# samtools/htslib

Hardware: NVIDIA H100
Metric: BGZF inflate + CRAM rANS decode GB/s at 1/2/4/8 H100 vs reference CPU (higher is better)
Workload: dtype u8

## Files before the change

htslib_b200/csrc/rans_nx16.cu:

```cuda
#include "hgpu_internal.h"
#include <stdio.h>

namespace {

constexpr uint32_t RANS_L = 1u << 15;
constexpr int SM_F      = 0;
constexpr int SM_CUM    = 1024;
constexpr int SM_ROWOF  = 2064;
constexpr int SM_SYMOF  = 2320;
constexpr int SM_RING   = 2576;
constexpr int SM_TAB    = 3088;
constexpr uint32_t GTAB_BYTES = 256u * 4096u + 256u * 256u * 4u;
constexpr uint32_t TBLBUF_BYTES = 256u * 1024u;

struct WarpScratch {
    uint8_t *tmp;
    uint8_t *planes;
    uint8_t *meta;
    uint8_t *tblbuf;
    uint8_t *gtab;
    uint32_t max_out;
    uint8_t *tab_base;
    uint32_t tab_cap;
    int pass;
    mutable bool defer;
    struct Hook *hook;
    bool compact = false;
};

struct Hook {
    int mode;
    bool taken;
    uint32_t order, N, shift, lb, ncol, ipos, U, R, row0, tab_bytes;
    const uint8_t *in; uint32_t in_len;
    uint8_t *out;
    uint8_t *lut; uint32_t *fb;
    uint16_t *Fcap;
};
constexpr int HOOK_X32 = 1, HOOK_N4 = 2;
constexpr int RC_HOOKED = 2;


__device__ int vget(const uint8_t *p, const uint8_t *end, uint32_t &v)
{
    const uint8_t *s = p;
    uint32_t acc = 0;
    uint8_t c;
    if (end - p >= 6) {
        int budget = 5;
        do { c = *p++; acc = (acc << 7) | (c & 0x7f); } while ((c & 0x80) && budget-- > 0);
    } else {
        if (p >= end) { v = 0; return 0; }
        do { c = *p++; acc = (acc << 7) | (c & 0x7f); } while ((c & 0x80) && p < end);
    }
    v = acc;
    return (int)(p - s);
}

__device__ int read_alphabet(const uint8_t *p, const uint8_t *end, uint32_t *F)
{
    const uint8_t *s = p;
    int run = 0, sym;
    if (p >= end) return 0;
    sym = *p++;
    if (sym == 0 && p + 2 >= end) return (int)(p - s);
    for (;;) {
        F[sym] = 1;
        if (p >= end) return 0;
        if (run == 0 && sym + 1 == *p) {
            if (p + 1 >= end) return 0;
            sym = *p++;
            run = *p++;
        } else if (run) {
// ... 355 lines not shown
            __syncwarp();
            ncol++;
        }
    }
    if (p == in) return -1;
    if (tot != 0 && tot != 4096) {
        int sh = 0;
        while (tot < 4096) { tot *= 2; sh++; }
        __syncwarp();
        for (uint32_t k = lane; k < ncol; k += 32) F[k] <<= sh;
        __syncwarp();
    }
    bool bad = false;
    for (uint32_t k = lane; k < ncol; k += 32) bad |= F[k] > 4096u;
    if (__any_sync(0xffffffffu, bad)) return -1;
    if (warp_cumsum(F, cum, (int)ncol) != 4096u) return -1;
    if (ncol == 0) return -1;
    Table t = place_table(smem, ws, 1, ncol, 12);
    if (ws.defer) return -1;
    fill_row(t, 0, F, cum, symof, N == 32);
    __syncwarp();
    uint32_t R;
    if (load_states(p, end, N, R)) return -1;
    uint32_t ipos = (uint32_t)(p - in) + 4 * N;
    if (top && ws.hook && t.in_smem && ws.hook->mode == (N == 32 ? HOOK_X32 : HOOK_N4)) {
        Hook &h = *ws.hook;
        if (h.Fcap && ncol <= 16) {
            __syncwarp();
            if (lane < 16) h.Fcap[lane] = lane < ncol ? (uint16_t)F[lane] : (uint16_t)0;
            if (lane == 0) h.Fcap[256] = 0;
            __syncwarp();
        }
        h.taken = true; h.order = 0; h.N = N; h.shift = 12; h.ncol = ncol; h.ipos = ipos; h.U = U; h.R = R; h.row0 = 0;
        h.in = in; h.in_len = in_len; h.out = out; h.lut = t.lut; h.fb = t.fb; h.lb = t.lb;
        h.tab_bytes = table_bytes(1, ncol, t.lb);
        return RC_HOOKED;
    }
    if (t.lb != t.shift) loop_order0<true, true>(smem, t, in, in_len, ipos, out, U, N, R);
    else if (t.in_smem)  loop_order0<true>(smem, t, in, in_len, ipos, out, U, N, R);
    else                 loop_order0<false>(smem, t, in, in_len, ipos, out, U, N, R);
    __syncwarp();
    return 0;
}

__device__ int dec_order1(uint8_t *smem, const WarpScratch &ws, const uint8_t *in, uint32_t in_len,
                          uint8_t *out, uint32_t U, uint32_t N, bool top = false)
{
    uint32_t *F = reinterpret_cast<uint32_t *>(smem + SM_F);
    uint32_t *cum = reinterpret_cast<uint32_t *>(smem + SM_CUM);
    uint8_t *rowof = smem + SM_ROWOF;
    uint8_t *symof = smem + SM_SYMOF;
    const uint32_t lane = hgpu_lane();
    if (in_len < (N == 4 ? 16u : 4u * N)) return -1;
    const uint8_t *p = in, *end = in + in_len, *tend = end, *after_tab = nullptr;
    const uint32_t shift = *p >> 4;
    if (*p++ & 1) {
        uint32_t usz, csz;
        p += vget(p, end, usz);
        p += vget(p, end, csz);
        if (csz > (uint32_t)(end - p)) return -1;
        if (usz > TBLBUF_BYTES) return -1;
        after_tab = p + csz;
        if (dec_order0(smem, ws, p, csz, ws.tblbuf, usz, 4)) return -1;
        __syncwarp();
        __threadfence_block();
        p = ws.tblbuf;
        tend = ws.tblbuf + usz;
    }
    if (shift != 10 && shift != 12) return -1;
    __syncwarp();
    for (int j = lane; j < 256; j += 32) { F[j] = 0; rowof[j] = 0xff; }
    __syncwarp();
    int n = read_alphabet(p, tend, F);
    if (!n) return -1;
    p += n;
    if (p >= tend) return -1;
    __syncwarp();
    uint32_t ncol = 0;
    bool zero_in_a0 = F[0] != 0;
    for (int j = 0; j < 256; j++) {
        if (F[j] || j == 0) {
            __syncwarp();
            if (lane == 0) { rowof[j] = (uint8_t)ncol; symof[ncol] = (uint8_t)j; }
            ncol++;
        }
    }
    __syncwarp();
    Table t = place_table(smem, ws, ncol, ncol, shift);
    if (ws.defer) return -1;
    const uint32_t total = 1u << shift;
    const uint8_t *rows_at = p;
build_rows:
    uint16_t *Fcap = (top && ws.hook && N == 32 && ncol <= 16) ? ws.hook->Fcap : nullptr;
    if (Fcap) {
        __syncwarp();
        for (uint32_t k = lane; k < 17 * 16; k += 32) Fcap[k] = k >= 256 ? (uint16_t)1 : (uint16_t)0;
        __syncwarp();
    }
    for (uint32_t r = 0; r < ncol; r++) {
        if (t.lb != shift && (r == 0 && !zero_in_a0)) goto need_full;
        if (r == 0 && !zero_in_a0) { fill_null_row(t, 0); continue; }
        const uint8_t *q = p;
        uint32_t T = 0;
        int dz = 0;
        if (q == tend) return -1;
        __syncwarp();
        for (uint32_t k = lane; k < ncol; k += 32) F[k] = 0;
        __syncwarp();
        for (uint32_t k = zero_in_a0 ? 0 : 1; k < ncol && q < tend; k++) {
            uint32_t f;
            if (dz) { f = 0; dz--; }
            else {
                q += vget(q, tend, f);
                if (f == 0) { if (q >= tend) return -1; dz = *q++; }
            }
            if (lane == 0) F[k] = f;
            T += f;
        }
        __syncwarp();
        if (q == p) return -1;
        p = q;
        if (!T && t.lb != shift) goto need_full;
        if (!T) { fill_null_row(t, r); continue; }
        if (T != total) {
            int sh = 0; uint32_t tt = T;
            while (tt < total) { tt *= 2; sh++; }
            for (uint32_t k = lane; k < ncol; k += 32) F[k] <<= sh;
            __syncwarp();
        }
        bool bad = false;
        for (uint32_t k = lane; k < ncol; k += 32) bad |= F[k] > total;
        if (__any_sync(0xffffffffu, bad)) return -1;
        if (warp_cumsum(F, cum, (int)ncol) != total) return -1;
        fill_row(t, r, F, cum, symof, false);
        if (Fcap) {
            if (lane < ncol) Fcap[r * 16 + lane] = (uint16_t)F[lane];
            if (lane == 0) Fcap[256 + r] = 0;
        }
        __syncwarp();
    }
    if (false) {
need_full:
        __syncwarp();
        t = place_table(smem, ws, ncol, ncol, shift, true);
        if (ws.defer) return -1;
        p = rows_at;
        goto build_rows;
    }
    __syncwarp();
    if (!t.in_smem) __threadfence_block();
    if (after_tab) p = after_tab;
    uint32_t R;
    if (load_states(p, end, N, R)) return -1;
    uint32_t ipos = (uint32_t)(p - in) + 4 * N;
    if (top && ws.hook && t.in_smem && ws.hook->mode == (N == 32 ? HOOK_X32 : HOOK_N4)) {
        Hook &h = *ws.hook;
        h.taken = true; h.order = 1; h.N = N; h.shift = shift; h.ncol = ncol; h.ipos = ipos; h.U = U; h.R = R; h.row0 = 0;
        h.in = in; h.in_len = in_len; h.out = out; h.lut = t.lut; h.fb = t.fb; h.lb = t.lb;
        h.tab_bytes = table_bytes(ncol, ncol, t.lb);
        return RC_HOOKED;
    }
    if (t.lb != shift) {
        if (N == 32) loop_order1<true, true, true>(smem, t, in, in_len, ipos, out, U, N, R, 0);
        else         loop_order1<true, false, true>(smem, t, in, in_len, ipos, out, U, N, R, 0);
    } else if (t.in_smem) {
        if (N == 32) loop_order1<true, true>(smem, t, in, in_len, ipos, out, U, N, R, 0);
        else         loop_order1<true, false>(smem, t, in, in_len, ipos, out, U, N, R, 0);
    } else           loop_order1<false, false>(smem, t, in, in_len, ipos, out, U, N, R, 0);
    __syncwarp();
    return 0;
}

__device__ int unpack_meta(const uint8_t *d, uint32_t len, uint8_t *map, int &per_byte)
{
    if (!len) return 0;
    uint32_t n = d[0] ? d[0] : 256, j = 1, c = 0;
    if (n <= 1) per_byte = 0;
    else if (n <= 2) per_byte = 8;
    else if (n <= 4) per_byte = 4;
    else if (n <= 16) per_byte = 2;
    else { per_byte = 1; return 1; }
    if (len <= 1) return 0;
    do { map[c++] = d[j++]; } while (c < n && j < len);
    return c < n ? 0 : (int)j;
}

__device__ int unpack(const uint8_t *d, uint64_t len, uint8_t *out, uint64_t olen, int per_byte,
                      const uint8_t *map)
{
    const uint32_t lane = hgpu_lane();
    if (per_byte == 1) { for (uint64_t i = lane; i < len; i += 32) out[i] = d[i]; return 0; }
    if (per_byte == 0) { for (uint64_t i = lane; i < olen; i += 32) out[i] = map[0]; return 0; }
// ... 408 lines not shown
        job = __shfl_sync(0xffffffffu, job, 0);
        if (job >= n) break;
        uint32_t got = 0;
        int rc = dec_4x8(gtab, in + in_off[job], in_len[job], out + out_off[job], out_len[job], got);
        __syncwarp();
        if (hgpu_lane() == 0) { status[job] = rc ? HGPU_RANS_ERR : HGPU_OK; got_len[job] = rc ? 0 : got; }
    }
}

}

static uint32_t g_f32_smem[64];

static uint32_t f32_smem(hgpu_ctx *ctx) { int d = ctx->device; return d >= 0 && d < 64 && g_f32_smem[d] ? g_f32_smem[d] : F32_SMEM + F32_LUT; }

static int rans_attrs(hgpu_ctx *ctx)
{
    static bool done[64];
    int dev = ctx->device;
    if (dev >= 0 && dev < 64 && done[dev]) return 0;
    {
        uint32_t *d_o = nullptr, base = 0;
        if (hgpu_check(cudaMalloc(&d_o, 4), "probe alloc")) return -1;
        rans_smem_probe_kernel<<<1, 32, 1024>>>(d_o);
        cudaError_t e = cudaMemcpy(&base, d_o, 4, cudaMemcpyDeviceToHost);
        cudaFree(d_o);
        if (hgpu_check(e, "smem probe")) return -1;
        uint32_t lut0 = (base + F32_WARPS * F32_RING + F32_LUT - 1) & ~(F32_LUT - 1);
        if (dev >= 0 && dev < 64) g_f32_smem[dev] = lut0 + F32_WARPS * (F32_LUT + F32_FB) - base;
    }
    if (hgpu_check(cudaFuncSetAttribute(rans_nx16_decode_kernel<1>, cudaFuncAttributeMaxDynamicSharedMemorySize, (int)(SM_TAB + 18 * 1024)), "rans smem attr") ||
        hgpu_check(cudaFuncSetAttribute(rans_prep32_kernel, cudaFuncAttributeMaxDynamicSharedMemorySize, (int)PREP_SMEM), "rans smem attr") ||
        hgpu_check(cudaFuncSetAttribute(rans_tile4_kernel, cudaFuncAttributeMaxDynamicSharedMemorySize, (int)T4_SMEM), "rans smem attr") ||
        hgpu_check(cudaFuncSetAttribute(rans_fast32_kernel, cudaFuncAttributeMaxDynamicSharedMemorySize, (int)f32_smem(ctx)), "rans smem attr"))
        return -1;
    if (dev >= 0 && dev < 64) done[dev] = true;
    return 0;
}

extern "C" uint32_t hgpu_rans_nx16_wave_size(hgpu_ctx *ctx)
{
    if (!ctx) return 0;
    if (cudaSetDevice(ctx->device) != cudaSuccess || rans_attrs(ctx)) return 0;
    int per_sm = 0;
    if (cudaOccupancyMaxActiveBlocksPerMultiprocessor(&per_sm, rans_fast32_kernel, F32_WARPS * 32, f32_smem(ctx)) != cudaSuccess) return 0;
    return (uint32_t)ctx->sm_count * (uint32_t)(per_sm < 1 ? 1 : per_sm) * F32_WARPS;
}

int hgpu_launch_rans_nx16(hgpu_ctx *ctx, const uint8_t *d_in, const uint64_t *d_in_off,
                          const uint32_t *d_in_len, uint32_t n, uint8_t *d_out,
                          const uint64_t *d_out_off, const uint32_t *d_out_len,
                          uint32_t *d_got_len, int32_t *d_status, uint32_t max_out_len,
                          cudaStream_t st)
{
    if (n == 0) return HGPU_OK;
    if (hgpu_check(cudaSetDevice(ctx->device), "cudaSetDevice") || rans_attrs(ctx)) return HGPU_ERR_CUDA;
    const uint32_t smem1 = SM_TAB + 18 * 1024;
    int per_prep = 0, per_t4 = 0, per_f32 = 0, per_gen = 0;
    if (hgpu_check(cudaOccupancyMaxActiveBlocksPerMultiprocessor(&per_prep, rans_prep32_kernel, 32, PREP_SMEM), "rans occupancy") ||
        hgpu_check(cudaOccupancyMaxActiveBlocksPerMultiprocessor(&per_t4, rans_tile4_kernel, 32, T4_SMEM), "rans occupancy") ||
        hgpu_check(cudaOccupancyMaxActiveBlocksPerMultiprocessor(&per_f32, rans_fast32_kernel, F32_WARPS * 32, f32_smem(ctx)), "rans occupancy") ||
        hgpu_check(cudaOccupancyMaxActiveBlocksPerMultiprocessor(&per_gen, rans_nx16_decode_kernel<1>, 32, smem1), "rans occupancy"))
        return HGPU_ERR_CUDA;
    auto grid_of = [&](int per_sm, uint32_t units) {
        uint32_t g = (uint32_t)ctx->sm_count * (uint32_t)(per_sm < 1 ? 1 : per_sm);
        return g > units ? (units ? units : 1u) : g;
    };
    const uint32_t g_prep = grid_of(per_prep, n), g_t4 = grid_of(per_t4, (n + 7) / 8 + 1);
    const uint32_t g_f32 = grid_of(per_f32, (n + F32_WARPS - 1) / F32_WARPS), g_gen = grid_of(per_gen, n);
    const size_t lists_b = ((size_t)2 * n * 4 + 255) & ~(size_t)255;
    const size_t jobs_b = (((size_t)n * sizeof(FastJob)) + 255) & ~(size_t)255;
    const size_t fixed = lists_b + 256 + jobs_b;
    const size_t mo = ((size_t)max_out_len + 255) & ~(size_t)255;
    const size_t per_small = TBLBUF_BYTES;
    const size_t per_gen_b = (3 * mo + 1024 + TBLBUF_BYTES + GTAB_BYTES + 255) & ~(size_t)255;
    size_t area = per_small * g_prep;
    if (per_small * g_t4 > area) area = per_small * g_t4;
    if (per_gen_b * g_gen > area) area = per_gen_b * g_gen;
    int rc = hgpu_ensure_scratch(ctx, fixed + area);
    if (rc) return rc;
    uint8_t *sc = ctx->d_scratch;
    uint32_t *list32 = reinterpret_cast<uint32_t *>(sc), *list4 = list32 + n;
    uint32_t *counts = reinterpret_cast<uint32_t *>(sc + lists_b);
    FastJob *jobs = reinterpret_cast<FastJob *>(sc + lists_b + 256);
    uint8_t *percta = sc + fixed;
    uint32_t *c_prep = hgpu_take_counter(ctx, st), *c_t4 = hgpu_take_counter(ctx, st), *c_f32 = hgpu_take_counter(ctx, st);
    uint32_t *c_gen = hgpu_take_counter(ctx, st), *njobs = hgpu_take_counter(ctx, st);
    if (!c_prep || !c_t4 || !c_f32 || !c_gen || !njobs) return HGPU_ERR_CUDA;
    rans_classify_kernel<<<1, 1024, 0, st>>>(d_in, d_in_off, d_in_len, n, d_status, list32, list4, counts);
    rans_prep32_kernel<<<g_prep, 32, PREP_SMEM, st>>>(d_in, d_in_off, d_in_len, list32, counts, d_out, d_out_off, d_out_len,
                                                      d_got_len, d_status, percta, per_small, max_out_len, jobs, njobs, c_prep);
    rans_tile4_kernel<<<g_t4, 32, T4_SMEM, st>>>(d_in, d_in_off, d_in_len, list4, counts, d_out, d_out_off, d_out_len,
                                                 d_got_len, d_status, percta, per_small, max_out_len, c_t4);
    rans_fast32_kernel<<<g_f32, F32_WARPS * 32, f32_smem(ctx), st>>>(jobs, njobs, d_in, d_in_off, d_in_len, d_out, d_out_off, d_out_len,
                                                                     d_status, c_f32, f32_smem(ctx));
    rans_nx16_decode_kernel<1><<<g_gen, 32, smem1, st>>>(d_in, d_in_off, d_in_len, n, d_out, d_out_off, d_out_len,
                                                         d_got_len, d_status, percta, per_gen_b,
                                                         max_out_len, 18 * 1024, c_gen);
    hgpu_count_launch(5);
    return hgpu_check(cudaGetLastError(), "rans launch");
}

extern "C" int hgpu_rans4x8_decode_batch_dev(hgpu_ctx *ctx, const uint8_t *d_in, const uint64_t *d_in_off,
        const uint32_t *d_in_len, uint32_t n, uint8_t *d_out, const uint64_t *d_out_off, const uint32_t *d_out_len,
        uint32_t *d_got_len, int32_t *d_status, void *stream)
{
    if (!ctx) { hgpu_set_error("null context"); return HGPU_ERR_ARG; }
    if (n == 0) return HGPU_OK;
    cudaStream_t st = stream ? (cudaStream_t)stream : ctx->stream;
    uint32_t grid = (uint32_t)ctx->sm_count * 16u;
    if (grid > n) grid = n;
    size_t per_cta = (GTAB_BYTES + 1024 + 255) & ~(size_t)255;
    int rc = hgpu_ensure_scratch(ctx, per_cta * grid);
    if (rc) return rc;
    uint32_t *counter = hgpu_take_counter(ctx, st);
    if (!counter) return HGPU_ERR_CUDA;
    rans_4x8_decode_kernel<<<grid, 32, 0, st>>>(d_in, d_in_off, d_in_len, n, d_out, d_out_off, d_out_len, d_got_len,
                                                d_status, ctx->d_scratch, per_cta, counter);
    hgpu_count_launch();
    return hgpu_check(cudaGetLastError(), "rans4x8 launch");
}
```

htslib_b200/csrc/rans_nx16_fast.cuh:

```cuda

constexpr int32_t RANS_PENDING = 3;

__global__ void __launch_bounds__(1024)
rans_classify_kernel(const uint8_t *__restrict__ in, const uint64_t *__restrict__ in_off,
                     const uint32_t *__restrict__ in_len, uint32_t n, int32_t *status,
                     uint32_t *list32, uint32_t *list4, uint32_t *counts )
{
    __shared__ uint32_t wsum[2][32];
    __shared__ uint32_t base[2];
    const uint32_t tid = threadIdx.x, lane = tid & 31, warp = tid >> 5;
    if (tid < 2) base[tid] = 0;
    __syncthreads();
    for (uint32_t i0 = 0; i0 < n; i0 += 1024) {
        uint32_t i = i0 + tid;
        int cls = 0;
        if (i < n) {
            uint32_t len = in_len[i];
            if (len >= 2) {
                uint8_t fmt = in[in_off[i]];
                if (!(fmt & 0xe8)) cls = (fmt & 0x04) ? 1 : 2;
            }
            status[i] = cls ? RANS_PENDING : RANS_DEFERRED;
        }
        uint32_t b1 = __ballot_sync(0xffffffffu, cls == 1), b2 = __ballot_sync(0xffffffffu, cls == 2);
        if (lane == 0) { wsum[0][warp] = __popc(b1); wsum[1][warp] = __popc(b2); }
        __syncthreads();
        uint32_t o1 = base[0], o2 = base[1];
        for (uint32_t w = 0; w < warp; w++) { o1 += wsum[0][w]; o2 += wsum[1][w]; }
        if (cls == 1) list32[o1 + __popc(b1 & hgpu_lanemask_lt())] = i;
        if (cls == 2) list4[o2 + __popc(b2 & hgpu_lanemask_lt())] = i;
        __syncthreads();
        if (tid == 0) {
            uint32_t t1 = 0, t2 = 0;
            for (int w = 0; w < 32; w++) { t1 += wsum[0][w]; t2 += wsum[1][w]; }
            base[0] += t1; base[1] += t2;
        }
        __syncthreads();
    }
    if (tid == 0) { counts[0] = base[0]; counts[1] = base[1]; }
}

struct __align__(16) FastJob {
    uint32_t job, ipos, shift, ncol, order, s0, U, hdr;
    uint32_t slen, pad[3];
    uint8_t  symof[8];
    uint8_t  ctx[32];
    uint32_t R[32];
    uint32_t prev[32];
    uint16_t F[64];
};

constexpr uint32_t F32_WARPS = 4, F32_LUT = 4096, F32_FB = 128, F32_RING = 768;
constexpr uint32_t F32_SMEM = F32_WARPS * (F32_LUT + F32_FB + F32_RING);
constexpr uint32_t F32_HEAD = 4;
constexpr uint32_t F32_MIN_U = 32 * 64;

__device__ bool fast32_emit(uint8_t *smem, const Hook &h, uint32_t job, uint32_t hdr, FastJob *jobs, uint32_t *njobs)
{
    const uint32_t lane = hgpu_lane();
    const uint16_t *Fc = h.Fcap;
    if (h.ncol > 16 || h.U < F32_MIN_U || h.lb != h.shift) return false;
    uint32_t emit = 0, nullrows = 0;
    const uint32_t rows = h.order ? h.ncol : 1;
    for (uint32_t r = 0; r < rows; r++) {
        if (h.order && Fc[256 + r]) { nullrows |= 1u << r; continue; }
        for (uint32_t k = 0; k < h.ncol; k++) if (Fc[r * 16 + k]) emit |= 1u << k;
    }
    const uint32_t ne = __popc(emit);
    if (ne == 0 || ne > 8) return false;
    if (h.order) {
        if ((ne << h.shift) > F32_LUT || ne > 4) return false;
        if (nullrows & emit) return false;
    }
    if (h.order && (nullrows & 1u)) return false;
    const uint8_t *symof = smem + SM_SYMOF;
    uint32_t R = h.R, ipos = h.ipos, acc = 0, krow = 0;
    if (h.order) {
        const uint32_t mask = (1u << h.shift) - 1, seg = h.U / 32;
        uint8_t *op = h.out + (size_t)lane * seg;
        uint8_t *ring = smem + SM_RING;
        WordRing wr;
        ring_init(ring, wr, h.in, h.in_len, ipos);
        uint32_t lrow = h.row0 << h.shift, frow = h.row0 * h.ncol;
        for (uint32_t s = 0; s < F32_HEAD; s++) {
            ring_ensure(ring, wr, ipos, 64);
            uint32_t m = R & mask;
            uint32_t k = h.lut[lrow + m];
            uint32_t e = h.fb[frow + k];
            uint32_t q = R >> h.shift;
            R = (e >> 20) * q + q + m - ((e >> 8) & 0xfffu);
            acc = __funnelshift_l(acc, e, 24);
            lrow = k << h.shift; frow = k * h.ncol; krow = k;
            renorm_safe(R, true, ring, wr, ipos, h.in_len);
            op[s] = (uint8_t)(acc >> 24);
        }
        __syncwarp();
        if (__any_sync(0xffffffffu, !(emit >> krow & 1u))) return false;
    }
    uint32_t slot = 0;
    if (lane == 0) slot = atomicAdd(njobs, 1u);
    slot = __shfl_sync(0xffffffffu, slot, 0);
    FastJob *fj = jobs + slot;
    if (lane == 0) {
        fj->job = job; fj->ipos = ipos; fj->shift = h.shift; fj->ncol = ne; fj->order = h.order;
        fj->s0 = h.order ? F32_HEAD : 0; fj->U = h.U; fj->hdr = hdr; fj->slen = h.in_len;
        uint32_t e = 0;
        for (uint32_t k = 0; k < h.ncol; k++) if (emit >> k & 1) fj->symof[e++] = symof[k];
        for (; e < 8; e++) fj->symof[e] = 0;
    }
    fj->R[lane] = R;
    fj->prev[lane] = acc;
    fj->ctx[lane] = (uint8_t)__popc(emit & ((1u << krow) - 1u));
    for (uint32_t idx = lane; idx < 64; idx += 32) {
        uint32_t re = idx >> 3, ke = idx & 7;
        uint16_t v = 0;
        if (re < (h.order ? ne : 1u) && ke < ne) {
            uint32_t r = h.order ? (uint32_t)__fns(emit, 0, re + 1) : 0u, k = (uint32_t)__fns(emit, 0, ke + 1);
            v = Fc[r * 16 + k];
        }
        fj->F[idx] = v;
    }
    return true;
}

__device__ __forceinline__ void lds_v2(uint32_t a, uint32_t &x, uint32_t &y)
{ asm volatile("ld.shared.v2.u32 {%0, %1}, [%2];" : "=r"(x), "=r"(y) : "r"(a) : "memory"); }
__device__ __forceinline__ void sts_u32(uint32_t a, uint32_t v) { asm volatile("st.shared.u32 [%0], %1;" :: "r"(a), "r"(v) : "memory"); }
__device__ __forceinline__ void sts_v2(uint32_t a, uint32_t x, uint32_t y) { asm volatile("st.shared.v2.u32 [%0], {%1, %2};" :: "r"(a), "r"(x), "r"(y) : "memory"); }

struct Ring32 {
    const uint8_t *in;
    uintptr_t lim;
    uint32_t a;
// ... 240 lines not shown
    for (;;) {
        uint32_t j = 0;
        if (hgpu_lane() == 0) j = atomicAdd(counter, 1u);
        j = __shfl_sync(0xffffffffu, j, 0);
        if (j >= n) break;
        const FastJob *fj = jobs + j;
        const uint32_t job = fj->job;
        const uint8_t *sin = in + in_off[job] + fj->hdr;
        const uint32_t slen = fj->slen;
        uint8_t *sout = out + out_off[job];
        const uint32_t U = fj->U;
        (void)out_len; (void)in_len;
        if ((fj->shift != 10 && fj->shift != 12) || fj->ncol == 0 || fj->ncol > 8 || (fj->order && (fj->ncol << fj->shift) > F32_LUT) ||
            (!fj->order && fj->shift != 12) || fj->hdr > in_len[job] || slen > in_len[job] - fj->hdr || fj->ipos > slen) {
            if (hgpu_lane() == 0) {
                printf("fast32: bad job %u: job=%u shift=%u ncol=%u order=%u hdr=%u slen=%u ipos=%u U=%u\n", j, job, fj->shift, fj->ncol,
                       fj->order, fj->hdr, slen, fj->ipos, U);
                status[job] = HGPU_RANS_ERR;
            }
            continue;
        }
        const bool sparse = (uint64_t)slen * 16 < U;
        if (fj->order) {
            if (sparse) fast32_stream<1, true>(fj, lut_a, fb_a, ring_a, sin, slen, sout, U);
            else        fast32_stream<1, false>(fj, lut_a, fb_a, ring_a, sin, slen, sout, U);
        } else {
            if (sparse) fast32_stream<0, true>(fj, lut_a, fb_a, ring_a, sin, slen, sout, U);
            else        fast32_stream<0, false>(fj, lut_a, fb_a, ring_a, sin, slen, sout, U);
        }
        if (hgpu_lane() == 0) status[job] = HGPU_OK;
    }
}

constexpr uint32_t PREP_TAB = 6656, PREP_SMEM = SM_TAB + PREP_TAB + 17 * 16 * 2;

__global__ void __launch_bounds__(32, 20)
rans_prep32_kernel(const uint8_t *__restrict__ in, const uint64_t *__restrict__ in_off,
                   const uint32_t *__restrict__ in_len, const uint32_t *__restrict__ list, const uint32_t *__restrict__ counts,
                   uint8_t *out, const uint64_t *__restrict__ out_off, const uint32_t *__restrict__ out_len,
                   uint32_t *got_len, int32_t *status, uint8_t *scratch, size_t scratch_per_cta,
                   uint32_t max_out, FastJob *jobs, uint32_t *njobs, uint32_t *counter)
{
    extern __shared__ __align__(16) uint8_t smem[];
    Hook hook;
    hook.mode = HOOK_X32;
    hook.Fcap = reinterpret_cast<uint16_t *>(smem + SM_TAB + PREP_TAB);
    WarpScratch ws;
    ws.tmp = ws.planes = ws.meta = ws.gtab = nullptr;
    ws.tblbuf = scratch + (size_t)blockIdx.x * scratch_per_cta;
    ws.max_out = max_out;
    ws.tab_base = smem + SM_TAB; ws.tab_cap = PREP_TAB;
    ws.pass = 0; ws.defer = false; ws.hook = &hook;
    const uint32_t n = counts[0];
    for (;;) {
        uint32_t idx = 0;
        if (hgpu_lane() == 0) idx = atomicAdd(counter, 1u);
        idx = __shfl_sync(0xffffffffu, idx, 0);
        if (idx >= n) break;
        const uint32_t job = list[idx];
        const uint8_t *sin = in + in_off[job];
        uint32_t got = 0;
        hook.taken = false;
        int rc = decode_stream(smem, ws, sin, in_len[job], out + out_off[job], out_len[job], got);
        __syncwarp();
        int32_t st;
        if (ws.defer) { st = RANS_DEFERRED; ws.defer = false; }
        else if (rc == RC_HOOKED) {
            if (fast32_emit(smem, hook, job, (uint32_t)(hook.in - sin), jobs, njobs)) st = RANS_PENDING;
            else {
                Table t; t.lut = hook.lut; t.fb = hook.fb; t.ncol = hook.ncol; t.shift = hook.shift; t.lb = hook.lb; t.in_smem = true;
                if (hook.lb != hook.shift) {
                    if (hook.order) loop_order1<true, true, true>(smem, t, hook.in, hook.in_len, hook.ipos, hook.out, hook.U, 32, hook.R, hook.row0);
                    else            loop_order0<true, true>(smem, t, hook.in, hook.in_len, hook.ipos, hook.out, hook.U, 32, hook.R);
                } else if (hook.order) loop_order1<true, true>(smem, t, hook.in, hook.in_len, hook.ipos, hook.out, hook.U, 32, hook.R, hook.row0);
                else            loop_order0<true>(smem, t, hook.in, hook.in_len, hook.ipos, hook.out, hook.U, 32, hook.R);
                __syncwarp();
                st = HGPU_OK;
            }
        } else st = rc ? HGPU_RANS_ERR : HGPU_OK;
        if (hgpu_lane() == 0) { status[job] = st; got_len[job] = (st == HGPU_OK || st == RANS_PENDING) ? got : 0; }
    }
}

struct Quad {
    uint32_t lut_a, fb_a, mask, shift, cs, rowsz, fstride, ipos, in_len, U, order, job, got;
    const uint8_t *in;
    uint8_t *out;
    uint32_t R[4];
};
constexpr uint32_t T4_POOL = 8192, T4_QUADS = SM_TAB + T4_POOL;
constexpr uint32_t T4_RING = 256;
constexpr uint32_t T4_RINGS = (T4_QUADS + 8 * (uint32_t)sizeof(Quad) + 15u) & ~15u, T4_SMEM = T4_RINGS + 8 * T4_RING;

__device__ __forceinline__ void quad_refill(uint32_t ring_a, const uint8_t *in, uint32_t in_len, uint32_t &loaded, uint32_t z, bool go)
{
    if (go) {
        const uint32_t off = loaded + 16u * z;
        const uintptr_t g = reinterpret_cast<uintptr_t>(in) + off, ga = g & ~(uintptr_t)3;
        const uintptr_t lim = (reinterpret_cast<uintptr_t>(in) + in_len + 3) & ~(uintptr_t)3;
        const uint32_t sh = (uint32_t)(g & 3) * 8u;
        uint32_t w[5];
// ... 166 lines not shown
```

include/htsgpu.h:

```cpp
#ifndef HTSGPU_H
#define HTSGPU_H

#include <stddef.h>
#include <stdint.h>

#ifdef __cplusplus
extern "C" {
#endif

#define HGPU_OK              0
#define HGPU_ERR_NODEVICE  (-100)
#define HGPU_ERR_CUDA      (-101)
#define HGPU_ERR_ARG       (-102)
#define HGPU_ERR_NOMEM     (-103)
#define HGPU_BGZF_ERR_ZLIB   (-1)
#define HGPU_BGZF_ERR_CRC    (-2)
#define HGPU_BGZF_ERR_HEADER (-3)
#define HGPU_BGZF_ERR_SPACE  (-4)
#define HGPU_RANS_ERR        (-1)
#define HGPU_TOK3_ERR        (-1)
#define HGPU_TOK3_ERR_LIMIT  (-5)

typedef struct hgpu_ctx hgpu_ctx;

// ... 13 lines not shown
        uint8_t *out, const uint64_t *out_off, const uint32_t *out_cap,
        uint32_t *out_len, int32_t *status);

int hgpu_bgzf_inflate_jobs_host(hgpu_ctx *ctx, uint32_t n, const uint8_t *const *comp, const uint32_t *comp_len,
        uint8_t *const *uncomp, uint32_t *uncomp_len, int32_t *status);

int hgpu_bgzf_compress_batch_dev(hgpu_ctx *ctx,
        const uint8_t *d_in, const uint64_t *d_in_off, const uint32_t *d_in_len, uint32_t n, int level,
        uint8_t *d_out, const uint64_t *d_out_off, uint32_t *d_out_len, int32_t *d_status, void *stream);

int hgpu_shard_range(uint64_t n_units, const uint32_t *unit_out_len, int world, int rank,
                     uint64_t *first, uint64_t *count, uint64_t *out_base);

long hgpu_bgzf_scan(const uint8_t *file, uint64_t file_len,
                    uint64_t *off, uint32_t *len, uint32_t *isize, long cap);

long hgpu_bgzf_gzi_entries(const uint64_t *off, const uint32_t *isize, long n, int terminating, uint64_t *caddr, uint64_t *uaddr, long cap);
long hgpu_bgzf_gzi_dump(const uint64_t *caddr, const uint64_t *uaddr, long n, uint8_t *out, size_t cap);
uint64_t hgpu_bgzf_useek(const uint64_t *caddr, const uint64_t *uaddr, long n, uint64_t u);
uint64_t hgpu_bgzf_utell(const uint64_t *caddr, const uint64_t *uaddr, long n, uint64_t voffset);

int hgpu_bgzf_inflate_file_host(hgpu_ctx *ctx, const uint8_t *file, uint64_t file_len,
                                uint8_t *out, uint64_t out_cap, uint64_t *out_len, long *bad_block);

uint32_t hgpu_crc32(hgpu_ctx *ctx, uint32_t crc, const void *buf, size_t len);
int hgpu_crc32_failed(void);

int hgpu_rans_nx16_decode_batch_dev(hgpu_ctx *ctx,
        const uint8_t *d_in, const uint64_t *d_in_off, const uint32_t *d_in_len, uint32_t n,
        uint8_t *d_out, const uint64_t *d_out_off, const uint32_t *d_out_len,
        uint32_t *d_got_len, int32_t *d_status, uint32_t max_out_len, void *stream);

uint32_t hgpu_rans_nx16_wave_size(hgpu_ctx *ctx);

int hgpu_rans_nx16_decode_batch_host(hgpu_ctx *ctx,
        const uint8_t *in, const uint64_t *in_off, const uint32_t *in_len, uint32_t n,
        uint8_t *out, const uint64_t *out_off, const uint32_t *out_len,
        uint32_t *got_len, int32_t *status);

int hgpu_rans4x8_decode_batch_dev(hgpu_ctx *ctx,
        const uint8_t *d_in, const uint64_t *d_in_off, const uint32_t *d_in_len, uint32_t n,
        uint8_t *d_out, const uint64_t *d_out_off, const uint32_t *d_out_len,
        uint32_t *d_got_len, int32_t *d_status, void *stream);

int hgpu_arith_decode_batch_dev(hgpu_ctx *ctx,
        const uint8_t *d_in, const uint64_t *d_in_off, const uint32_t *d_in_len, uint32_t n,
        uint8_t *d_out, const uint64_t *d_out_off, const uint32_t *d_out_len,
        uint32_t *d_got_len, int32_t *d_status, uint32_t max_out_len, void *stream);

uint32_t hgpu_rans4x8_compress_bound(uint32_t size);
int hgpu_rans4x8_encode_batch_dev(hgpu_ctx *ctx,
        const uint8_t *d_in, const uint64_t *d_in_off, const uint32_t *d_in_len, const uint32_t *d_order,
        uint32_t n, uint8_t *d_out, const uint64_t *d_out_off, const uint32_t *d_out_cap,
        uint32_t *d_out_len, int32_t *d_status, void *stream);

uint32_t hgpu_arith_compress_bound(uint32_t size, int order);
int hgpu_arith_encode_batch_dev(hgpu_ctx *ctx,
        const uint8_t *d_in, const uint64_t *d_in_off, const uint32_t *d_in_len, const uint32_t *d_order,
        uint32_t n, uint8_t *d_out, const uint64_t *d_out_off, const uint32_t *d_out_cap,
        uint32_t *d_out_len, int32_t *d_status, uint32_t max_in_len, void *stream);

typedef struct hgpu_cram_block {
    uint64_t data_off;
    uint32_t comp_size, uncomp_size;
    int32_t  content_id;
    uint8_t  method, content_type;
// ... 209 lines not shown
```

Baseline: 183.5.

## Route wide-alphabet order-1 X32 rANS streams to a dedicated wide32 decode kernel

Adds a new wide32 kernel for order-1 32-way rANS streams whose alphabet holds 17-65 symbols. The prep kernel stashes the frequency matrix in the output buffer and emits a job; the new kernel then builds a compact LUT in shared memory and decodes with warp-cooperative renormalisation and vectorised stores. Previously these streams fell back to the generic decoder. The change also moves head byte writes in fast32_emit and adds global route counters with a query API. The costs are an extra launch, extra atomics, and a frequency stash written into the output buffer.

```diff
diff --git a/htslib_b200/csrc/rans_nx16.cu b/htslib_b200/csrc/rans_nx16.cu
--- a/htslib_b200/csrc/rans_nx16.cu
+++ b/htslib_b200/csrc/rans_nx16.cu
@@ -36,9 +36,15 @@
     uint8_t *out;
     uint8_t *lut; uint32_t *fb;
     uint16_t *Fcap;
+    const uint16_t *wcap;
 };
 constexpr int HOOK_X32 = 1, HOOK_N4 = 2;
 constexpr int RC_HOOKED = 2;
+
+constexpr uint32_t W32_NCOL = 65;
+__device__ __forceinline__ uint16_t *w32_stash(uint8_t *out)
+{ return reinterpret_cast<uint16_t *>((reinterpret_cast<uintptr_t>(out) + 3u) & ~(uintptr_t)3u); }
+__device__ __forceinline__ bool w32_fits(uint32_t ncol, uint32_t U) { return ncol <= W32_NCOL && U >= 4u + 2u * ncol * ncol; }
 
 
 __device__ int vget(const uint8_t *p, const uint8_t *end, uint32_t &v)
@@ -460,7 +466,7 @@
             __syncwarp();
         }
         h.taken = true; h.order = 0; h.N = N; h.shift = 12; h.ncol = ncol; h.ipos = ipos; h.U = U; h.R = R; h.row0 = 0;
-        h.in = in; h.in_len = in_len; h.out = out; h.lut = t.lut; h.fb = t.fb; h.lb = t.lb;
+        h.in = in; h.in_len = in_len; h.out = out; h.lut = t.lut; h.fb = t.fb; h.lb = t.lb; h.wcap = nullptr;
         h.tab_bytes = table_bytes(1, ncol, t.lb);
         return RC_HOOKED;
     }
@@ -514,8 +520,13 @@
         }
     }
     __syncwarp();
-    Table t = place_table(smem, ws, ncol, ncol, shift);
-    if (ws.defer) return -1;
+    uint16_t *Wcap = (top && ws.hook && ws.hook->mode == HOOK_X32 && N == 32 && w32_fits(ncol, U)) ? w32_stash(out) : nullptr;
+    const bool table = !(Wcap && ncol > 16);
+    Table t = {};
+    if (table) {
+        t = place_table(smem, ws, ncol, ncol, shift);
+        if (ws.defer) return -1;
+    }
     const uint32_t total = 1u << shift;
     const uint8_t *rows_at = p;
 build_rows:
@@ -526,8 +537,12 @@
         __syncwarp();
     }
     for (uint32_t r = 0; r < ncol; r++) {
-        if (t.lb != shift && (r == 0 && !zero_in_a0)) goto need_full;
-        if (r == 0 && !zero_in_a0) { fill_null_row(t, 0); continue; }
+        if (Wcap) {
+            for (uint32_t k = lane; k < ncol; k += 32) Wcap[r * ncol + k] = 0;
+            __syncwarp();
+        }
+        if (table && t.lb != shift && (r == 0 && !zero_in_a0)) goto need_full;
+        if (r == 0 && !zero_in_a0) { if (table) fill_null_row(t, 0); continue; }
         const uint8_t *q = p;
         uint32_t T = 0;
         int dz = 0;
@@ -548,8 +563,8 @@
         __syncwarp();
         if (q == p) return -1;
         p = q;
-        if (!T && t.lb != shift) goto need_full;
-        if (!T) { fill_null_row(t, r); continue; }
+        if (!T && table && t.lb != shift) goto need_full;
+        if (!T) { if (table) fill_null_row(t, r); continue; }
         if (T != total) {
             int sh = 0; uint32_t tt = T;
             while (tt < total) { tt *= 2; sh++; }
@@ -560,11 +575,12 @@
         for (uint32_t k = lane; k < ncol; k += 32) bad |= F[k] > total;
         if (__any_sync(0xffffffffu, bad)) return -1;
         if (warp_cumsum(F, cum, (int)ncol) != total) return -1;
-        fill_row(t, r, F, cum, symof, false);
+        if (table) fill_row(t, r, F, cum, symof, false);
         if (Fcap) {
             if (lane < ncol) Fcap[r * 16 + lane] = (uint16_t)F[lane];
             if (lane == 0) Fcap[256 + r] = 0;
         }
+        if (Wcap) for (uint32_t k = lane; k < ncol; k += 32) Wcap[r * ncol + k] = (uint16_t)F[k];
         __syncwarp();
     }
     if (false) {
@@ -576,16 +592,16 @@
         goto build_rows;
     }
     __syncwarp();
-    if (!t.in_smem) __threadfence_block();
+    if (table && !t.in_smem) __threadfence_block();
     if (after_tab) p = after_tab;
     uint32_t R;
     if (load_states(p, end, N, R)) return -1;
     uint32_t ipos = (uint32_t)(p - in) + 4 * N;
-    if (top && ws.hook && t.in_smem && ws.hook->mode == (N == 32 ? HOOK_X32 : HOOK_N4)) {
+    if (top && ws.hook && (!table || t.in_smem) && ws.hook->mode == (N == 32 ? HOOK_X32 : HOOK_N4)) {
         Hook &h = *ws.hook;
         h.taken = true; h.order = 1; h.N = N; h.shift = shift; h.ncol = ncol; h.ipos = ipos; h.U = U; h.R = R; h.row0 = 0;
-        h.in = in; h.in_len = in_len; h.out = out; h.lut = t.lut; h.fb = t.fb; h.lb = t.lb;
-        h.tab_bytes = table_bytes(ncol, ncol, t.lb);
+        h.in = in; h.in_len = in_len; h.out = out; h.lut = t.lut; h.fb = t.fb; h.lb = t.lb; h.wcap = Wcap;
+        h.tab_bytes = table ? table_bytes(ncol, ncol, t.lb) : 0u;
         return RC_HOOKED;
     }
     if (t.lb != shift) {
@@ -1060,7 +1076,8 @@
     if (hgpu_check(cudaFuncSetAttribute(rans_nx16_decode_kernel<1>, cudaFuncAttributeMaxDynamicSharedMemorySize, (int)(SM_TAB + 18 * 1024)), "rans smem attr") ||
         hgpu_check(cudaFuncSetAttribute(rans_prep32_kernel, cudaFuncAttributeMaxDynamicSharedMemorySize, (int)PREP_SMEM), "rans smem attr") ||
         hgpu_check(cudaFuncSetAttribute(rans_tile4_kernel, cudaFuncAttributeMaxDynamicSharedMemorySize, (int)T4_SMEM), "rans smem attr") ||
-        hgpu_check(cudaFuncSetAttribute(rans_fast32_kernel, cudaFuncAttributeMaxDynamicSharedMemorySize, (int)f32_smem(ctx)), "rans smem attr"))
+        hgpu_check(cudaFuncSetAttribute(rans_fast32_kernel, cudaFuncAttributeMaxDynamicSharedMemorySize, (int)f32_smem(ctx)), "rans smem attr") ||
+        hgpu_check(cudaFuncSetAttribute(rans_wide32_kernel, cudaFuncAttributeMaxDynamicSharedMemorySize, (int)W32_SMEM), "rans smem attr"))
         return -1;
     if (dev >= 0 && dev < 64) done[dev] = true;
     return 0;
@@ -1084,10 +1101,11 @@
     if (n == 0) return HGPU_OK;
     if (hgpu_check(cudaSetDevice(ctx->device), "cudaSetDevice") || rans_attrs(ctx)) return HGPU_ERR_CUDA;
     const uint32_t smem1 = SM_TAB + 18 * 1024;
-    int per_prep = 0, per_t4 = 0, per_f32 = 0, per_gen = 0;
+    int per_prep = 0, per_t4 = 0, per_f32 = 0, per_w32 = 0, per_gen = 0;
     if (hgpu_check(cudaOccupancyMaxActiveBlocksPerMultiprocessor(&per_prep, rans_prep32_kernel, 32, PREP_SMEM), "rans occupancy") ||
         hgpu_check(cudaOccupancyMaxActiveBlocksPerMultiprocessor(&per_t4, rans_tile4_kernel, 32, T4_SMEM), "rans occupancy") ||
         hgpu_check(cudaOccupancyMaxActiveBlocksPerMultiprocessor(&per_f32, rans_fast32_kernel, F32_WARPS * 32, f32_smem(ctx)), "rans occupancy") ||
+        hgpu_check(cudaOccupancyMaxActiveBlocksPerMultiprocessor(&per_w32, rans_wide32_kernel, 32, W32_SMEM), "rans occupancy") ||
         hgpu_check(cudaOccupancyMaxActiveBlocksPerMultiprocessor(&per_gen, rans_nx16_decode_kernel<1>, 32, smem1), "rans occupancy"))
         return HGPU_ERR_CUDA;
     auto grid_of = [&](int per_sm, uint32_t units) {
@@ -1095,10 +1113,11 @@
         return g > units ? (units ? units : 1u) : g;
     };
     const uint32_t g_prep = grid_of(per_prep, n), g_t4 = grid_of(per_t4, (n + 7) / 8 + 1);
-    const uint32_t g_f32 = grid_of(per_f32, (n + F32_WARPS - 1) / F32_WARPS), g_gen = grid_of(per_gen, n);
+    const uint32_t g_f32 = grid_of(per_f32, (n + F32_WARPS - 1) / F32_WARPS), g_w32 = grid_of(per_w32, n), g_gen = grid_of(per_gen, n);
     const size_t lists_b = ((size_t)2 * n * 4 + 255) & ~(size_t)255;
     const size_t jobs_b = (((size_t)n * sizeof(FastJob)) + 255) & ~(size_t)255;
-    const size_t fixed = lists_b + 256 + jobs_b;
+    const size_t wjobs_b = (((size_t)n * sizeof(WideJob)) + 255) & ~(size_t)255;
+    const size_t fixed = lists_b + 256 + jobs_b + wjobs_b;
     const size_t mo = ((size_t)max_out_len + 255) & ~(size_t)255;
     const size_t per_small = TBLBUF_BYTES;
     const size_t per_gen_b = (3 * mo + 1024 + TBLBUF_BYTES + GTAB_BYTES + 255) & ~(size_t)255;
@@ -1111,22 +1130,36 @@
     uint32_t *list32 = reinterpret_cast<uint32_t *>(sc), *list4 = list32 + n;
     uint32_t *counts = reinterpret_cast<uint32_t *>(sc + lists_b);
     FastJob *jobs = reinterpret_cast<FastJob *>(sc + lists_b + 256);
+    WideJob *wjobs = reinterpret_cast<WideJob *>(sc + lists_b + 256 + jobs_b);
     uint8_t *percta = sc + fixed;
     uint32_t *c_prep = hgpu_take_counter(ctx, st), *c_t4 = hgpu_take_counter(ctx, st), *c_f32 = hgpu_take_counter(ctx, st);
     uint32_t *c_gen = hgpu_take_counter(ctx, st), *njobs = hgpu_take_counter(ctx, st);
-    if (!c_prep || !c_t4 || !c_f32 || !c_gen || !njobs) return HGPU_ERR_CUDA;
+    uint32_t *c_w32 = hgpu_take_counter(ctx, st), *nwide = hgpu_take_counter(ctx, st);
+    if (!c_prep || !c_t4 || !c_f32 || !c_gen || !njobs || !c_w32 || !nwide) return HGPU_ERR_CUDA;
     rans_classify_kernel<<<1, 1024, 0, st>>>(d_in, d_in_off, d_in_len, n, d_status, list32, list4, counts);
     rans_prep32_kernel<<<g_prep, 32, PREP_SMEM, st>>>(d_in, d_in_off, d_in_len, list32, counts, d_out, d_out_off, d_out_len,
-                                                      d_got_len, d_status, percta, per_small, max_out_len, jobs, njobs, c_prep);
+                                                      d_got_len, d_status, percta, per_small, max_out_len, jobs, njobs, wjobs, nwide, c_prep);
     rans_tile4_kernel<<<g_t4, 32, T4_SMEM, st>>>(d_in, d_in_off, d_in_len, list4, counts, d_out, d_out_off, d_out_len,
                                                  d_got_len, d_status, percta, per_small, max_out_len, c_t4);
     rans_fast32_kernel<<<g_f32, F32_WARPS * 32, f32_smem(ctx), st>>>(jobs, njobs, d_in, d_in_off, d_in_len, d_out, d_out_off, d_out_len,
                                                                      d_status, c_f32, f32_smem(ctx));
+    rans_wide32_kernel<<<g_w32, 32, W32_SMEM, st>>>(wjobs, nwide, d_in, d_in_off, d_in_len, d_out, d_out_off, d_status, c_w32);
     rans_nx16_decode_kernel<1><<<g_gen, 32, smem1, st>>>(d_in, d_in_off, d_in_len, n, d_out, d_out_off, d_out_len,
                                                          d_got_len, d_status, percta, per_gen_b,
                                                          max_out_len, 18 * 1024, c_gen);
-    hgpu_count_launch(5);
+    hgpu_count_launch(6);
     return hgpu_check(cudaGetLastError(), "rans launch");
+}
+
+extern "C" int hgpu_rans_nx16_x32_routes(hgpu_ctx *ctx, uint64_t *narrow, uint64_t *wide)
+{
+    if (!ctx || !narrow || !wide) { hgpu_set_error("null argument"); return HGPU_ERR_ARG; }
+    unsigned long long r[2] = {0, 0};
+    if (hgpu_check(cudaSetDevice(ctx->device), "cudaSetDevice") || hgpu_check(cudaDeviceSynchronize(), "synchronize") ||
+        hgpu_check(cudaMemcpyFromSymbol(r, g_x32_routes, sizeof(r)), "route counters"))
+        return HGPU_ERR_CUDA;
+    *narrow = r[0]; *wide = r[1];
+    return HGPU_OK;
 }
 
 extern "C" int hgpu_rans4x8_decode_batch_dev(hgpu_ctx *ctx, const uint8_t *d_in, const uint64_t *d_in_off,
diff --git a/htslib_b200/csrc/rans_nx16_fast.cuh b/htslib_b200/csrc/rans_nx16_fast.cuh
--- a/htslib_b200/csrc/rans_nx16_fast.cuh
+++ b/htslib_b200/csrc/rans_nx16_fast.cuh
@@ -49,6 +49,8 @@
     uint32_t prev[32];
     uint16_t F[64];
 };
+
+__device__ unsigned long long g_x32_routes[2];
 
 constexpr uint32_t F32_WARPS = 4, F32_LUT = 4096, F32_FB = 128, F32_RING = 768;
 constexpr uint32_t F32_SMEM = F32_WARPS * (F32_LUT + F32_FB + F32_RING);
@@ -92,13 +94,13 @@
             acc = __funnelshift_l(acc, e, 24);
             lrow = k << h.shift; frow = k * h.ncol; krow = k;
             renorm_safe(R, true, ring, wr, ipos, h.in_len);
-            op[s] = (uint8_t)(acc >> 24);
         }
         __syncwarp();
         if (__any_sync(0xffffffffu, !(emit >> krow & 1u))) return false;
+        for (uint32_t s = 0; s < F32_HEAD; s++) op[s] = (uint8_t)(acc >> (8 * s));
     }
     uint32_t slot = 0;
-    if (lane == 0) slot = atomicAdd(njobs, 1u);
+    if (lane == 0) { slot = atomicAdd(njobs, 1u); atomicAdd(&g_x32_routes[0], 1ull); }
     slot = __shfl_sync(0xffffffffu, slot, 0);
     FastJob *fj = jobs + slot;
     if (lane == 0) {
@@ -405,6 +407,227 @@
     }
 }
 
+struct __align__(16) WideJob {
+    uint32_t job, ipos, shift, ncol, lb, U, hdr, slen;
+    uint32_t R[32];
+    uint8_t  symof[80];
+};
+
+constexpr uint32_t W32_TAB = 21072;
+constexpr uint32_t W32_SYM = 128;
+constexpr uint32_t W32_SMEM = 256 + W32_TAB + W32_SYM + F32_RING;
+
+__device__ __forceinline__ uint32_t w32_tab_bytes(uint32_t ncol, uint32_t lb) { return (((ncol << lb) + 15u) & ~15u) + 4u * ncol * ncol; }
+
+__device__ bool wide32_emit(const uint8_t *smem, const Hook &h, uint32_t job, uint32_t hdr, WideJob *jobs, uint32_t *njobs)
+{
+    const uint32_t lane = hgpu_lane(), n = h.ncol;
+    const uint16_t *F = h.wcap;
+    if (h.U < F32_MIN_U) return false;
+    __syncwarp();
+    uint32_t nul[3], emit[3];
+#pragma unroll
+    for (int g = 0; g < 3; g++) {
+        const uint32_t r = 32u * g + lane;
+        bool z = r < n;
+        for (uint32_t k = 0; z && k < n; k++) z = F[r * n + k] == 0;
+        nul[g] = __ballot_sync(0xffffffffu, z);
+    }
+#pragma unroll
+    for (int g = 0; g < 3; g++) {
+        const uint32_t k = 32u * g + lane;
+        bool e = false;
+        for (uint32_t r = 0; k < n && !e && r < n; r++)
+            e = !((r < 32 ? nul[0] : r < 64 ? nul[1] : nul[2]) >> (r & 31) & 1u) && F[r * n + k] != 0;
+        emit[g] = __ballot_sync(0xffffffffu, e);
+    }
+    const uint32_t ne = __popc(emit[0]) + __popc(emit[1]) + __popc(emit[2]);
+    if (ne == 0 || ne > 64) return false;
+    if (nul[0] & 1u) return false;
+    if ((nul[0] & emit[0]) | (nul[1] & emit[1]) | (nul[2] & emit[2])) return false;
+    uint32_t lb = 8;
+    while (lb > 6 && w32_tab_bytes(n, lb) > W32_TAB) lb--;
+    uint32_t slot = 0;
+    if (lane == 0) { slot = atomicAdd(njobs, 1u); atomicAdd(&g_x32_routes[1], 1ull); }
+    slot = __shfl_sync(0xffffffffu, slot, 0);
+    WideJob *wj = jobs + slot;
+    if (lane == 0) {
+        wj->job = job; wj->ipos = h.ipos; wj->shift = h.shift; wj->ncol = n; wj->lb = lb; wj->U = h.U;
+        wj->hdr = hdr; wj->slen = h.in_len;
+    }
+    wj->R[lane] = h.R;
+    for (uint32_t k = lane; k < sizeof(wj->symof); k += 32) wj->symof[k] = k < n ? smem[SM_SYMOF + k] : 0;
+    return true;
+}
+
+__device__ __forceinline__ void sts_u8(uint32_t a, uint32_t v) { asm volatile("st.shared.u8 [%0], %1;" :: "r"(a), "r"(v) : "memory"); }
+
+__device__ __forceinline__ void wide32_stream(const WideJob *wj, uint32_t lut_a, uint32_t sym_a, uint32_t ring_a,
+                                              const uint8_t *in, uint32_t in_len, uint8_t *out)
+{
+    const uint32_t lane = hgpu_lane();
+    const uint32_t shift = wj->shift, ncol = wj->ncol, lb = wj->lb, U = wj->U;
+    const uint32_t mask = (1u << shift) - 1u, cs = shift - lb, nbm = (1u << lb) - 1u, rowsz = 1u << lb;
+    const uint32_t fstride = 4u * ncol, kmax = ncol - 1u;
+    const uint32_t fb_a = lut_a + (((ncol << lb) + 15u) & ~15u);
+    {
+        const uint16_t *F = w32_stash(out);
+        for (uint32_t r = lane; r < ncol; r += 32) {
+            const uint32_t lrow = lut_a + (r << lb);
+            uint32_t c = 0;
+            for (uint32_t k = 0; k < ncol; k++) {
+                const uint32_t f = F[r * ncol + k];
+                sts_u32(fb_a + r * fstride + 4u * k, c | f << 16);
+                const uint32_t b0 = (c + (1u << cs) - 1u) >> cs, b1 = (c + f + (1u << cs) - 1u) >> cs;
+                for (uint32_t b = b0; b < b1; b++) sts_u8(lrow + b, k);
+                c += f;
+            }
+            if (c == 0) for (uint32_t b = 0; b < rowsz; b++) sts_u8(lrow + b, 0);
+        }
+        for (uint32_t k = lane; k < ncol; k += 32) sts_u8(sym_a + k, wj->symof[k]);
+    }
+    uint32_t R = wj->R[lane];
+    __syncwarp();
+    Ring32 rg;
+    rg.in = in; rg.lim = (reinterpret_cast<uintptr_t>(in) + in_len + 3) & ~(uintptr_t)3;
+    rg.a = ring_a; rg.v = 0; rg.loaded = 0; rg.pos0 = wj->ipos;
+    ring32_fill(rg);
+    __syncwarp();
+    const uint32_t lt = hgpu_lanemask_lt();
+
+#define W32_SYMBOL                                                                                         \
+        uint32_t k_ = lds_u8(lop3_and_or(R >> cs, nbm, lrow));                                             \
+        const uint32_t k1_ = min(k_ + 1u, kmax);                                                           \
+        uint32_t e_ = lds_u32(frow + 4u * k_);                                                             \
+        const uint32_t e1_ = lds_u32(frow + 4u * k1_);                                                     \
+        const uint32_t m_ = R & mask;                                                                      \
+        if (m_ >= (e1_ & 0xffffu)) { e_ = e1_; k_ = k1_; }                                                 \
+        while (__any_sync(0xffffffffu, m_ >= (e_ & 0xffffu) + (e_ >> 16))) {                               \
+            if (m_ >= (e_ & 0xffffu) + (e_ >> 16)) { k_++; e_ = lds_u32(frow + 4u * k_); }                 \
+        }                                                                                                  \
+        R = (e_ >> 16) * (R >> shift) + m_ - (e_ & 0xffffu);                                               \
+        lrow = mad_lo(k_, rowsz, lut_a); frow = mad_lo(k_, fstride, fb_a);
+#define W32_RENORM_FAST                                                                                    \
+        {                                                                                                  \
+            const bool p_ = R < RANS_L;                                                                    \
+            const uint32_t bal_ = __ballot_sync(0xffffffffu, p_);                                          \
+            const uint32_t w_ = lds_u16(relA + 2u * __popc(bal_ & lt));                                    \
+            if (p_) R = __byte_perm(w_, R, 0x5410);                                                        \
+            relA += 2u * __popc(bal_);                                                                     \
+        }
+
+    const uint32_t seg = U / 32;
+    uint8_t *op = out + (size_t)lane * seg;
+    uint32_t lrow = lut_a, frow = fb_a;
+    uint32_t s = 0, prevB = 0;
+    for (; s < F32_HEAD; s++) {
+        ring32_fill(rg);
+        W32_SYMBOL
+        const uint32_t b_ = lds_u8(sym_a + k_);
+        op[s] = (uint8_t)b_;
+        prevB = __funnelshift_r(prevB, b_, 8);
+        renorm32_safe(R, true, rg, in_len);
+    }
+    const uint32_t ph = (uint32_t)(reinterpret_cast<uintptr_t>(op) + s) & 3u;
+    const uint32_t shamt = 32u - 8u * ph;
+    uint32_t *wp = reinterpret_cast<uint32_t *>(op + s - ph);
+    uint32_t relA = rg.a + (rg.v & 511u);
+#define W32_GROUP(WREG)                                                                                  \
+        {                                                                                                  \
+            const uint32_t g0 = relA;                                                                      \
+            uint32_t B = 0;                                                                                \
+            _Pragma("unroll")                                                                              \
+            for (int j = 0; j < 4; j++) {                                                                  \
+                W32_SYMBOL                                                                                 \
+                B = __funnelshift_r(B, lds_u8(sym_a + k_), 8);                                             \
+                W32_RENORM_FAST                                                                            \
+            }                                                                                              \
+            WREG = __funnelshift_rc(prevB, B, shamt);                                                      \
+            prevB = B;                                                                                     \
+            rg.v += relA - g0;                                                                             \
+            if (relA >= rg.a + 512u) relA -= 512u;                                                         \
+            ring32_fill(rg);                                                                               \
+        }
+    if (s + 16 <= seg && rg.pos0 + rg.v + 1024u <= in_len) {
+        const uint32_t q0 = (uint32_t)(reinterpret_cast<uintptr_t>(wp) >> 2) & 3u;
+        const bool p0 = q0 == 3u, p1 = q0 == 2u, p2 = q0 == 1u, p3 = q0 == 0u;
+        uint32_t W0, W1, W2, W3;
+        W32_GROUP(W0) wp[0] = W0;
+        W32_GROUP(W1) wp[1] = W1;
+        W32_GROUP(W2) wp[2] = W2;
+        W32_GROUP(W3) wp[3] = W3;
+        wp += 4; s += 16;
+        while (s + 16 <= seg && rg.pos0 + rg.v + 1024u <= in_len) {
+            W32_GROUP(W0) if (p0) *reinterpret_cast<uint4 *>(wp - 3) = make_uint4(W1, W2, W3, W0);
+            W32_GROUP(W1) if (p1) *reinterpret_cast<uint4 *>(wp - 2) = make_uint4(W2, W3, W0, W1);
+            W32_GROUP(W2) if (p2) *reinterpret_cast<uint4 *>(wp - 1) = make_uint4(W3, W0, W1, W2);
+            W32_GROUP(W3) if (p3) *reinterpret_cast<uint4 *>(wp) = make_uint4(W0, W1, W2, W3);
+            wp += 4; s += 16;
+        }
+        wp[-3] = W1; wp[-2] = W2; wp[-1] = W3;
+    }
+    while (s + 4 <= seg && rg.pos0 + rg.v + 256u <= in_len) {
+        uint32_t W;
+        W32_GROUP(W)
+        *wp++ = W;
+        s += 4;
+    }
+#undef W32_GROUP
+    op[s - 1] = (uint8_t)(prevB >> 24);
+    op[s - 2] = (uint8_t)(prevB >> 16);
+    op[s - 3] = (uint8_t)(prevB >> 8);
+    for (; s < seg; s++) {
+        ring32_fill(rg);
+        W32_SYMBOL
+        op[s] = (uint8_t)lds_u8(sym_a + k_);
+        renorm32_safe(R, true, rg, in_len);
+    }
+    const bool last = lane == 31;
+    for (uint32_t s2 = seg * 32; s2 < U; s2++) {
+        ring32_fill(rg);
+        const uint32_t Rk = R, lk = lrow, fk = frow;
+        W32_SYMBOL
+        if (last) out[s2] = (uint8_t)lds_u8(sym_a + k_);
+        else { R = Rk; lrow = lk; frow = fk; }
+        renorm32_safe(R, last, rg, in_len);
+    }
+#undef W32_SYMBOL
+#undef W32_RENORM_FAST
+    __syncwarp();
+}
+
+__global__ void __launch_bounds__(32)
+rans_wide32_kernel(const WideJob *__restrict__ jobs, const uint32_t *__restrict__ njobs,
+                   const uint8_t *__restrict__ in, const uint64_t *__restrict__ in_off,
+                   const uint32_t *__restrict__ in_len, uint8_t *out, const uint64_t *__restrict__ out_off,
+                   int32_t *status, uint32_t *counter)
+{
+    extern __shared__ __align__(16) uint8_t smem[];
+    const uint32_t sbase = (uint32_t)__cvta_generic_to_shared(smem);
+    const uint32_t lut_a = (sbase + 255u) & ~255u, sym_a = lut_a + W32_TAB, ring_a = sym_a + W32_SYM;
+    const uint32_t n = *njobs;
+    for (;;) {
+        uint32_t j = 0;
+        if (hgpu_lane() == 0) j = atomicAdd(counter, 1u);
+        j = __shfl_sync(0xffffffffu, j, 0);
+        if (j >= n) break;
+        const WideJob *wj = jobs + j;
+        const uint32_t job = wj->job, ncol = wj->ncol, lb = wj->lb;
+        if ((wj->shift != 10 && wj->shift != 12) || ncol == 0 || ncol > W32_NCOL || lb < 6 || lb > 8 ||
+            w32_tab_bytes(ncol, lb) > W32_TAB || wj->U < F32_MIN_U || !w32_fits(ncol, wj->U) ||
+            wj->hdr > in_len[job] || wj->slen > in_len[job] - wj->hdr || wj->ipos > wj->slen) {
+            if (hgpu_lane() == 0) {
+                printf("wide32: bad job %u: job=%u shift=%u ncol=%u lb=%u hdr=%u slen=%u ipos=%u U=%u\n", j, job, wj->shift, ncol, lb,
+                       wj->hdr, wj->slen, wj->ipos, wj->U);
+                status[job] = HGPU_RANS_ERR;
+            }
+            continue;
+        }
+        wide32_stream(wj, lut_a, sym_a, ring_a, in + in_off[job] + wj->hdr, wj->slen, out + out_off[job]);
+        if (hgpu_lane() == 0) status[job] = HGPU_OK;
+    }
+}
+
 constexpr uint32_t PREP_TAB = 6656, PREP_SMEM = SM_TAB + PREP_TAB + 17 * 16 * 2;
 
 __global__ void __launch_bounds__(32, 20)
@@ -412,7 +635,7 @@
                    const uint32_t *__restrict__ in_len, const uint32_t *__restrict__ list, const uint32_t *__restrict__ counts,
                    uint8_t *out, const uint64_t *__restrict__ out_off, const uint32_t *__restrict__ out_len,
                    uint32_t *got_len, int32_t *status, uint8_t *scratch, size_t scratch_per_cta,
-                   uint32_t max_out, FastJob *jobs, uint32_t *njobs, uint32_t *counter)
+                   uint32_t max_out, FastJob *jobs, uint32_t *njobs, WideJob *wjobs, uint32_t *nwide, uint32_t *counter)
 {
     extern __shared__ __align__(16) uint8_t smem[];
     Hook hook;
@@ -439,7 +662,10 @@
         int32_t st;
         if (ws.defer) { st = RANS_DEFERRED; ws.defer = false; }
         else if (rc == RC_HOOKED) {
-            if (fast32_emit(smem, hook, job, (uint32_t)(hook.in - sin), jobs, njobs)) st = RANS_PENDING;
+            const uint32_t hdr = (uint32_t)(hook.in - sin);
+            if (fast32_emit(smem, hook, job, hdr, jobs, njobs)) st = RANS_PENDING;
+            else if (hook.wcap && wide32_emit(smem, hook, job, hdr, wjobs, nwide)) st = RANS_PENDING;
+            else if (!hook.lut) st = RANS_DEFERRED;
             else {
                 Table t; t.lut = hook.lut; t.fb = hook.fb; t.ncol = hook.ncol; t.shift = hook.shift; t.lb = hook.lb; t.in_smem = true;
                 if (hook.lb != hook.shift) {
diff --git a/include/htsgpu.h b/include/htsgpu.h
--- a/include/htsgpu.h
+++ b/include/htsgpu.h
@@ -69,6 +69,8 @@
         uint32_t *d_got_len, int32_t *d_status, uint32_t max_out_len, void *stream);
 
 uint32_t hgpu_rans_nx16_wave_size(hgpu_ctx *ctx);
+
+int hgpu_rans_nx16_x32_routes(hgpu_ctx *ctx, uint64_t *narrow, uint64_t *wide);
 
 int hgpu_rans_nx16_decode_batch_host(hgpu_ctx *ctx,
         const uint8_t *in, const uint64_t *in_off, const uint32_t *in_len, uint32_t n,
```

Result: no change. 183.5 (median of 6 runs) (+0.0%).
